# angelvillar96/STLPose

Hardware: AMD Instinct MI355X
Metric: images/sec/GPU HRNet-W32 384x288 train step; PCKh@0.5 parity (higher is better)
Workload: dtype f16/bf16; 1 GPU; HRNet-W32 384x288 bs=32/GPU train step (fwd+MSE+bwd+Adam), random-init weights; global_batch=32, parallelism=dp1

## Files before the change

stlpose_amd/csrc/elementwise.hip:

```cpp
#include "common.cuh"

namespace {

template <typename T>
__device__ __forceinline__ void load8(const void* base, size_t elem, float* f) {
    if constexpr (sizeof(T) == 2) {
        unpack<T>(ldg16((const char*)base + elem * 2), f);
    } else {
        unpack<float>(ldg16((const char*)base + elem * 4), f);
        unpack<float>(ldg16((const char*)base + elem * 4 + 16), f + 4);
    }
}
template <typename T>
__device__ __forceinline__ void store8(void* base, size_t elem, const float* f) {
    if constexpr (sizeof(T) == 2) {
        stg16((char*)base + elem * 2, pack<T>(f));
    } else {
        stg16((char*)base + elem * 4, pack<float>(f));
        stg16((char*)base + elem * 4 + 16, pack<float>(f + 4));
    }
}

template <int NS>
__device__ __forceinline__ void flush_sets(float (*acc)[8], float* red, int C, int VPC, double* const* dst,
// ... 209 lines not shown
                if (t < p.nbn) {
#pragma unroll
                    for (int j = 0; j < 8; ++j)
                        acc[1 + t][j] += d[j] * (y[t][j] - mu[(t * 2) * C + c0 + j]) * mu[(t * 2 + 1) * C + c0 + j];
                }
            }
        }
    }
    if (p.nbn > 0) {
        double* dst[5];
        int which[5];
#pragma unroll
        for (int t = 0; t < 4; ++t) {
            if (t < p.nbn) {
                dst[0] = p.rstats[t], which[0] = 0;
                dst[1] = p.rstats[t], which[1] = 1;
                float two[2][8];
#pragma unroll
                for (int j = 0; j < 8; ++j) two[0][j] = acc[0][j], two[1][j] = acc[1 + t][j];
                flush_sets<2>(two, red, C, VPC, dst, which, 2);
            }
        }
    }
}

template <typename T, typename TY, int SHIFT>
__global__ __launch_bounds__(256) void upsample_bwd_kernel(const stl_upbwd p) {
    extern __shared__ __attribute__((aligned(16))) char smem[];
    const int C = p.C, VPC = C >> 3;
    float* mu = reinterpret_cast<float*>(smem);
    float* red = mu + 2 * C;
    for (int c = threadIdx.x; c < C; c += blockDim.x) {
        float m, r;
        bn_mean_rstd(p.bn, c, C, m, r);
        mu[c] = m, mu[C + c] = r;
    }
    __syncthreads();
    float acc[2][8];
#pragma unroll
    for (int s = 0; s < 2; ++s)
#pragma unroll
        for (int j = 0; j < 8; ++j) acc[s][j] = 0.f;
    constexpr int F = 1 << SHIFT;
    const uint32_t Wh = (uint32_t)p.W << SHIFT, Hh = (uint32_t)p.H << SHIFT;
    const uint32_t total = (uint32_t)p.B * p.H * p.W * VPC;
    const int cg = threadIdx.x % VPC, c0 = cg * 8;
    for (uint32_t v = blockIdx.x * blockDim.x + threadIdx.x; v < total; v += gridDim.x * blockDim.x) {
        const uint32_t pi = v / (uint32_t)VPC;
        const uint32_t by = pi / (uint32_t)p.W, x = pi - by * p.W;
        const uint32_t b = by / (uint32_t)p.H, y = by - b * p.H;
        float yv[8];
        load8<TY>(p.bn.x, (size_t)pi * C + c0, yv);
        float s[8];
#pragma unroll
        for (int j = 0; j < 8; ++j) s[j] = 0.f;
        const size_t row0 = ((size_t)(b * Hh + y * F) * Wh + x * F) * C + c0;
#pragma unroll(SHIFT == 1 ? 2 : 1)
        for (int dy = 0; dy < F; ++dy) {
            float d[F][8];
#pragma unroll
            for (int dx = 0; dx < F; ++dx) load8<T>(p.du, row0 + ((size_t)dy * Wh + dx) * C, d[dx]);
#pragma unroll
            for (int dx = 0; dx < F; ++dx)
#pragma unroll
                for (int j = 0; j < 8; ++j) s[j] += d[dx][j];
        }
#pragma unroll
        for (int j = 0; j < 8; ++j) s[j] = round_to<T>(s[j]);
        store8<T>(p.dt, (size_t)pi * C + c0, s);
#pragma unroll
        for (int j = 0; j < 8; ++j) {
            acc[0][j] += s[j];
            acc[1][j] += s[j] * (yv[j] - mu[c0 + j]) * mu[C + c0 + j];
        }
    }
    double* dst[2] = {p.rstats, p.rstats};
    int which[2] = {0, 1};
    flush_sets<2>(acc, red, C, VPC, dst, which, 2);
}

template <typename T>
__global__ __launch_bounds__(256) void patch_kernel(const float* img, void* out, int B, int H, int W, int Ho, int Wo,
                                                    int stride, const float* mean3, const float* std3) {
    const size_t total = (size_t)B * Ho * Wo * 4;
    float mean[3] = {0.f, 0.f, 0.f}, istd[3] = {1.f, 1.f, 1.f};
    if (mean3) {
#pragma unroll
        for (int c = 0; c < 3; ++c) mean[c] = mean3[c], istd[c] = 1.f / std3[c];
    }
    for (size_t v = (size_t)blockIdx.x * 256 + threadIdx.x; v < total; v += (size_t)gridDim.x * 256) {
        const size_t pi = v >> 2;
        const int part = (int)(v & 3);
        const int ox = (int)(pi % Wo);
        const size_t by = pi / Wo;
        const int oy = (int)(by % Ho), b = (int)(by / Ho);
        float f[8];
#pragma unroll
        for (int j = 0; j < 8; ++j) {
            const int kk = part * 8 + j;
            float val = 0.f;
            if (kk < 27) {
                const int tap = kk / 3, c = kk - tap * 3;
                const int iy = oy * stride + tap / 3 - 1, ix = ox * stride + tap % 3 - 1;
                if (iy >= 0 && iy < H && ix >= 0 && ix < W) {
                    val = img[(((size_t)b * 3 + c) * H + iy) * W + ix];
                    if (mean3) val = (val - mean[c]) / std3[c];
                }
            }
            f[j] = val;
        }
        (void)istd;
        store8<T>(out, pi * 32 + part * 8, f);
    }
}

template <typename T, int S>
__global__ __launch_bounds__(256) void patch_bwd_kernel(const void* dp, float* dimg, int B, int H, int W, int Ho, int Wo,
                                                        const float* std3) {
    constexpr int R0 = S == 1 ? -1 : 0;
    const size_t total = (size_t)B * Ho * Wo;
    for (size_t pi = (size_t)blockIdx.x * 256 + threadIdx.x; pi < total; pi += (size_t)gridDim.x * 256) {
        const int ox = (int)(pi % Wo);
        const size_t by = pi / Wo;
        const int oy = (int)(by % Ho), b = (int)(by / Ho);
        float acc[3][S][S];
#pragma unroll
        for (int c = 0; c < 3; ++c)
#pragma unroll
            for (int u = 0; u < S; ++u)
#pragma unroll
                for (int v = 0; v < S; ++v) acc[c][u][v] = 0.f;
#pragma unroll
        for (int ry = R0; ry <= 1; ++ry) {
#pragma unroll
            for (int rx = R0; rx <= 1; ++rx) {
                const int qy = oy + ry, qx = ox + rx;
                if (qy < 0 || qy >= Ho || qx < 0 || qx >= Wo) continue;
                const size_t row = (((size_t)b * Ho + qy) * Wo + qx) * 32;
                float f[32];
#pragma unroll
                for (int q = 0; q < 4; ++q) load8<T>(dp, row + q * 8, f + q * 8);
#pragma unroll
                for (int ky = 0; ky < 3; ++ky) {
                    const int dy = ry * S + ky - 1;
                    if (dy < 0 || dy >= S) continue;
#pragma unroll
                    for (int kx = 0; kx < 3; ++kx) {
                        const int dx = rx * S + kx - 1;
                        if (dx < 0 || dx >= S) continue;
#pragma unroll
                        for (int c = 0; c < 3; ++c) acc[c][dy][dx] += f[(ky * 3 + kx) * 3 + c];
                    }
                }
            }
        }
#pragma unroll
        for (int c = 0; c < 3; ++c) {
            const float sd = std3 ? std3[c] : 1.f;
#pragma unroll
            for (int u = 0; u < S; ++u) {
                const int iy = oy * S + u;
                if (iy >= H) continue;
                float* dst = dimg + (((size_t)b * 3 + c) * H + iy) * W + (size_t)ox * S;
                if (S == 2 && (W & 1) == 0) {
                    *reinterpret_cast<float2*>(dst) = make_float2(acc[c][u][0] / sd, acc[c][u][S - 1] / sd);
                } else {
#pragma unroll
                    for (int v = 0; v < S; ++v)
                        if (ox * S + v < W) dst[v] = acc[c][u][v] / sd;
                }
            }
        }
    }
}

template <typename T, int J>
__global__ __launch_bounds__(256) void head_fwd_kernel(const void* x, const float* w, const float* bias, float* out,
                                                       int B, int HW, int Ci) {
    extern __shared__ __attribute__((aligned(16))) char smem[];
    float* sw = reinterpret_cast<float*>(smem);
    for (int e = threadIdx.x; e < J * Ci; e += 256) sw[e] = w[e];
    __syncthreads();
    const size_t P = (size_t)B * HW;
    for (size_t pi = (size_t)blockIdx.x * 256 + threadIdx.x; pi < P; pi += (size_t)gridDim.x * 256) {
        float o[J];
#pragma unroll
        for (int j = 0; j < J; ++j) o[j] = bias ? bias[j] : 0.f;
        for (int c0 = 0; c0 < Ci; c0 += 8) {
            float f[8];
            load8<T>(x, pi * Ci + c0, f);
#pragma unroll
            for (int j = 0; j < J; ++j)
#pragma unroll
                for (int q = 0; q < 8; ++q) o[j] = fmaf(f[q], sw[j * Ci + c0 + q], o[j]);
        }
        const size_t b = pi / HW, hw = pi - b * HW;
#pragma unroll
        for (int j = 0; j < J; ++j) out[(b * J + j) * HW + hw] = o[j];
    }
}

template <typename T, int J, typename TY = T>
__global__ __launch_bounds__(256) void head_bwd_kernel(const void* x, const float* w, const float* dout, void* dx,
                                                       float* partial, int B, int HW, int Ci) {
    extern __shared__ __attribute__((aligned(16))) char smem[];
    constexpr int SDP = 260;
    constexpr int NTMAX = 4;
    float* sw = reinterpret_cast<float*>(smem);
    float* sd = sw + ((J * Ci + 3) & ~3);
    float* sx = sd + J * SDP;
    const int tid = threadIdx.x, lane = tid & 63, wave = tid >> 6, r16 = lane & 15, g = lane >> 4;
    const int nt_n = Ci >> 4;
    for (int e = tid; e < J * Ci; e += 256) sw[e] = w[e];
    const int nel = J * Ci + J;
    f32x4 acc[2][NTMAX];
#pragma unroll
    for (int mt = 0; mt < 2; ++mt)
#pragma unroll
        for (int nt = 0; nt < NTMAX; ++nt) acc[mt][nt] = f32x4{0.f, 0.f, 0.f, 0.f};
    float bsum = 0.f;
    const size_t P = (size_t)B * HW;
    const size_t nchunk = (P + 255) / 256;
    for (size_t ch = blockIdx.x; ch < nchunk; ch += gridDim.x) {
        const size_t pi = ch * 256 + tid;
        __syncthreads();
        float d[J];
        if (pi < P) {
            const size_t b = pi / HW, hw = pi - b * HW;
#pragma unroll
            for (int j = 0; j < J; ++j) d[j] = dout[(b * J + j) * HW + hw];
        } else {
#pragma unroll
            for (int j = 0; j < J; ++j) d[j] = 0.f;
        }
#pragma unroll
        for (int j = 0; j < J; ++j) sd[j * SDP + tid] = d[j];
        for (int c0 = 0; c0 < Ci; c0 += 8) {
            float f[8], gx[8];
            if (pi < P) {
                load8<TY>(x, pi * Ci + c0, f);
            } else {
#pragma unroll
                for (int q = 0; q < 8; ++q) f[q] = 0.f;
            }
#pragma unroll
            for (int q = 0; q < 8; ++q) {
                sx[tid * (Ci + 1) + c0 + q] = f[q];
                float s = 0.f;
#pragma unroll
                for (int j = 0; j < J; ++j) s = fmaf(d[j], sw[j * Ci + c0 + q], s);
                gx[q] = s;
            }
            if (pi < P) store8<T>(dx, pi * Ci + c0, gx);
        }
        __syncthreads();
        const int px0 = wave * 64 + g;
        const float* arow0 = sd + r16 * SDP + px0;
        const float* arow1 = sd + (16 + r16 < J ? 16 + r16 : 0) * SDP + px0;
        const bool a1ok = 16 + r16 < J;
        const float* brow = sx + (size_t)px0 * (Ci + 1) + r16;
#pragma unroll 4
        for (int ks = 0; ks < 16; ++ks) {
            const float a0 = arow0[4 * ks];
            const float a1 = a1ok ? arow1[4 * ks] : 0.f;
#pragma unroll
            for (int nt = 0; nt < NTMAX; ++nt) {
                if (nt < nt_n) {
                    const float bv = brow[(size_t)4 * ks * (Ci + 1) + nt * 16];
                    acc[0][nt] = __builtin_amdgcn_mfma_f32_16x16x4f32(a0, bv, acc[0][nt], 0, 0, 0);
                    acc[1][nt] = __builtin_amdgcn_mfma_f32_16x16x4f32(a1, bv, acc[1][nt], 0, 0, 0);
                }
            }
        }
        if (tid < 4 * J) {
            const float* r = sd + (tid >> 2) * SDP + (tid & 3) * 64;
            float s = 0.f;
#pragma unroll
            for (int q = 0; q < 16; ++q) {
                const float4 v = *reinterpret_cast<const float4*>(r + 4 * q);
                s += (v.x + v.y) + (v.z + v.w);
            }
            bsum += s;
        }
    }
    __syncthreads();
    f32x4* red = reinterpret_cast<f32x4*>(sx);
#pragma unroll
    for (int mt = 0; mt < 2; ++mt)
#pragma unroll
        for (int nt = 0; nt < NTMAX; ++nt)
            if (nt < nt_n) red[(wave * 2 * NTMAX + mt * NTMAX + nt) * 64 + lane] = acc[mt][nt];
    float* bred = reinterpret_cast<float*>(red + 4 * 2 * NTMAX * 64);
    if (tid < 4 * J) bred[tid] = bsum;
    __syncthreads();
    for (int e = tid; e < nel; e += 256) {
        float s;
        if (e < J * Ci) {
            const int j = e / Ci, c = e - j * Ci;
            const int tile = (j >> 4) * NTMAX + (c >> 4), ln = 16 * ((j & 15) >> 2) + (c & 15), rr = j & 3;
            s = (red[(0 * 2 * NTMAX + tile) * 64 + ln][rr] + red[(1 * 2 * NTMAX + tile) * 64 + ln][rr]) +
                (red[(2 * 2 * NTMAX + tile) * 64 + ln][rr] + red[(3 * 2 * NTMAX + tile) * 64 + ln][rr]);
        } else {
            const int j = e - J * Ci;
            s = (bred[4 * j] + bred[4 * j + 1]) + (bred[4 * j + 2] + bred[4 * j + 3]);
        }
        partial[(size_t)blockIdx.x * nel + e] = s;
    }
}

__global__ __launch_bounds__(256) void mse_kernel(const float* o, const float* t, const float* tw, float* dout,
                                                  double* partial, size_t n, int HW, float gs) {
    double acc = 0.0;
    for (size_t i = (size_t)blockIdx.x * 256 + threadIdx.x; i < n; i += (size_t)gridDim.x * 256) {
        const float w = tw[i / HW];
        const float d = (o[i] - t[i]) * w;
        acc += (double)d * (double)d;
        if (dout) dout[i] = d * w * gs;
    }
    __shared__ double sred[4];
    acc = wave_sum_d(acc);
    if ((threadIdx.x & 63) == 0) sred[threadIdx.x >> 6] = acc;
    __syncthreads();
    if (threadIdx.x == 0) partial[blockIdx.x] = sred[0] + sred[1] + sred[2] + sred[3];
}

__global__ __launch_bounds__(256) void sum_partials_kernel(const double* partial, int n, double scale, float* out, int accumulate) {
    double acc = 0.0;
    for (int i = threadIdx.x; i < n; i += 256) acc += partial[i];
    __shared__ double sred[4];
    acc = wave_sum_d(acc);
    if ((threadIdx.x & 63) == 0) sred[threadIdx.x >> 6] = acc;
    __syncthreads();
    if (threadIdx.x == 0) {
        const double s = (sred[0] + sred[1] + sred[2] + sred[3]) * scale;
        out[0] = (float)((accumulate ? (double)out[0] : 0.0) + s);
    }
}

__global__ __launch_bounds__(256) void argmax_kernel(const float* hm, int32_t* idx, float* maxval, float* preds, int H, int W) {
    __shared__ float sv[4];
    __shared__ int si[4];
    const float* row = hm + (size_t)blockIdx.x * H * W;
    float bv;
    int bi;
    block_argmax(row, H * W, bv, bi, sv, si);
    if (threadIdx.x == 0) {
        if (idx) idx[blockIdx.x] = bi;
        maxval[blockIdx.x] = bv;
        const float m = bv > 0.f ? 1.f : 0.f;
        preds[2 * blockIdx.x] = (float)(bi % W) * m;
        preds[2 * blockIdx.x + 1] = (float)(bi / W) * m;
    }
}

__global__ __launch_bounds__(256) void final_preds_kernel(const float* hm, const float* center, const float* scale,
                                                          float* preds, float* maxval, int J, int H, int W) {
    __shared__ float sv[4];
    __shared__ int si[4];
    const float* row = hm + (size_t)blockIdx.x * H * W;
    float bv;
    int bi;
    block_argmax(row, H * W, bv, bi, sv, si);
    if (threadIdx.x == 0) {
        const float m = bv > 0.f ? 1.f : 0.f;
        float cx = (float)(bi % W) * m, cy = (float)(bi / W) * m;
        const int px = (int)floorf(cx + 0.5f), py = (int)floorf(cy + 0.5f);
        if (1 < px && px < W - 1 && 1 < py && py < H - 1) {
            const float dx = row[py * W + px + 1] - row[py * W + px - 1];
            const float dy = row[(py + 1) * W + px] - row[(py - 1) * W + px];
            cx += (dx > 0.f) ? 0.25f : (dx < 0.f ? -0.25f : 0.f);
            cy += (dy > 0.f) ? 0.25f : (dy < 0.f ? -0.25f : 0.f);
        }
        const int b = blockIdx.x / J;
        const double s = (double)W / ((double)scale[2 * b] * 200.0);
        preds[2 * blockIdx.x] = (float)(((double)cx - 0.5 * W) / s + (double)center[2 * b]);
        preds[2 * blockIdx.x + 1] = (float)(((double)cy - 0.5 * H) / s + (double)center[2 * b + 1]);
        maxval[blockIdx.x] = bv;
    }
}

__global__ __launch_bounds__(256) void flip_merge_kernel(const float* a, const float* bf, float* out, const int32_t* perm,
                                                         int J, int H, int W, size_t n) {
    for (size_t i = (size_t)blockIdx.x * 256 + threadIdx.x; i < n; i += (size_t)gridDim.x * 256) {
        const int x = (int)(i % W);
        const size_t r = i / W;
        const int y = (int)(r % H);
        const size_t bj = r / H;
        const int j = (int)(bj % J);
        const size_t b = bj / J;
        const int xs = x > 0 ? x - 1 : 0;
        const float f = bf[((b * J + perm[j]) * H + y) * W + (W - 1 - xs)];
        out[i] = 0.5f * (a[i] + f);
    }
}

__global__ __launch_bounds__(256) void flip_merge_bwd_kernel(const float* g, float* da, float* dbf, const int32_t* perm,
                                                             int J, int H, int W, size_t n) {
    for (size_t i = (size_t)blockIdx.x * 256 + threadIdx.x; i < n; i += (size_t)gridDim.x * 256) {
        const int x = (int)(i % W);
        const size_t r = i / W;
// ... 550 lines not shown
    for (int t = 0; t < p.nterms; ++t) flat = flat && p.t[t].shift == 0;
    const bool big = flat && total >= ((size_t)1 << 21) && ((size_t)grid.x * 256) % (size_t)(p.C / 8) == 0;
#define STL_FUSE(TT)                                                                   \
    do {                                                                               \
        if (big) STL_LAUNCH(fuse_flat_big_kernel<TT>, grid, dim3(256), lds, ST, p);    \
        else STL_LAUNCH(fuse_fwd_kernel<TT>, grid, dim3(256), lds, ST, p);             \
    } while (0)
    if (p.dtype == STL_BF16)
        STL_FUSE(__bf16);
    else if (p.dtype == STL_F16)
        STL_FUSE(f16);
    else
        STL_FUSE(float);
#undef STL_FUSE
    STL_LAUNCH_CHECK("fuse_forward");
    return 0;
}

static int stat_block(int C) {
    const int vpc = C / 8;
    return vpc * (256 / vpc);
}

extern "C" int stl_fuse_backward(const stl_fuse_bwd* pp, void* stream) {
    const stl_fuse_bwd& p = *pp;
    STL_CHECK(p.C % 8 == 0 && p.C > 0 && p.C <= 1024, "fuse_bwd: C=%d", p.C);
    STL_CHECK(p.ngrads >= 1 && p.ngrads <= 4 && p.nbn >= 0 && p.nbn <= 4, "fuse_bwd: ngrads/nbn");
    STL_CHECK(!p.relu || p.z, "fuse_bwd: relu needs z");
    for (int t = 0; t < p.nbn; ++t) STL_CHECK(p.bn[t].x && (p.bn[t].stats || (p.bn[t].rmean && p.bn[t].rvar)) && p.rstats[t], "fuse_bwd: bn term %d incomplete", t);
    const int bd = stat_block(p.C);
    const size_t total = (size_t)p.B * p.H * p.W * (p.C / 8);
    int cap = (int)(total / (size_t)(bd * 16));
    cap = cap < 256 ? 256 : (cap > 1024 ? 1024 : cap);
    int nb = nblocks_for(total, bd, cap);
    const size_t lds = (size_t)(p.nbn > 0 ? p.nbn : 1) * 2 * p.C * 4 + (size_t)bd * 2 * 8 * 4;
    STL_CHECK(p.ydtype == 0 || p.ydtype == p.dtype || (p.dtype == STL_BF16 && p.ydtype == STL_F16), "fuse_bwd: ydtype %d does not go with dtype %d", p.ydtype, p.dtype);
    if (p.dtype == STL_BF16 && p.ydtype == STL_F16)
        STL_LAUNCH((fuse_bwd_kernel<__bf16, f16>), dim3(nb), dim3(bd), lds, ST, p);
    else if (p.dtype == STL_BF16)
        STL_LAUNCH(fuse_bwd_kernel<__bf16>, dim3(nb), dim3(bd), lds, ST, p);
    else
        STL_LAUNCH(fuse_bwd_kernel<float>, dim3(nb), dim3(bd), lds, ST, p);
    STL_LAUNCH_CHECK("fuse_backward");
    return 0;
}

extern "C" int stl_upsample_backward(const stl_upbwd* pp, void* stream) {
    const stl_upbwd& p = *pp;
    STL_CHECK(p.C % 8 == 0 && p.C > 0 && p.C <= 1024, "upsample_bwd: C=%d", p.C);
    STL_CHECK(p.shift >= 1 && p.shift <= 3, "upsample_bwd: shift %d (1 .. 3)", p.shift);
    STL_CHECK(p.du && p.dt && p.bn.x && (p.bn.stats || (p.bn.rmean && p.bn.rvar)) && p.rstats, "upsample_bwd: null pointer");
    const int bd = stat_block(p.C);
    const size_t total = (size_t)p.B * p.H * p.W * (p.C / 8);
    int cap = (int)(total / (size_t)(bd * 16));
    cap = cap < 256 ? 256 : (cap > 1024 ? 1024 : cap);
    int nb = nblocks_for(total, bd, cap);
    const size_t lds = (size_t)2 * p.C * 4 + (size_t)bd * 2 * 8 * 4;
    STL_CHECK(p.ydtype == 0 || p.ydtype == p.dtype || (p.dtype == STL_BF16 && p.ydtype == STL_F16), "upsample_bwd: ydtype %d does not go with dtype %d", p.ydtype, p.dtype);
    STL_CHECK(total * 8 < (1ull << 31) && ((size_t)p.B * (p.H << p.shift) * (p.W << p.shift) * p.C) < (1ull << 32),
              "upsample_bwd: tensors of 2^31 or more elements are not supported (32-bit index arithmetic)");
#define STL_UP(TT, TYY)                                                                                         \
    do {                                                                                                        \
        if (p.shift == 1) STL_LAUNCH((upsample_bwd_kernel<TT, TYY, 1>), dim3(nb), dim3(bd), lds, ST, p);        \
        else if (p.shift == 2) STL_LAUNCH((upsample_bwd_kernel<TT, TYY, 2>), dim3(nb), dim3(bd), lds, ST, p);   \
        else if (p.shift == 3) STL_LAUNCH((upsample_bwd_kernel<TT, TYY, 3>), dim3(nb), dim3(bd), lds, ST, p);   \
        else return stl_set_error("upsample_bwd: shift %d has no instantiation (1 .. 3)", p.shift);             \
    } while (0)
    if (p.dtype == STL_BF16 && p.ydtype == STL_F16)
        STL_UP(__bf16, f16);
    else if (p.dtype == STL_BF16)
        STL_UP(__bf16, __bf16);
    else
        STL_UP(float, float);
#undef STL_UP
    STL_LAUNCH_CHECK("upsample_backward");
    return 0;
}

extern "C" int stl_patch3x3(int dtype, const float* img, void* out, int B, int H, int W, int stride, const float* mean3,
                            const float* std3, void* stream) {
    STL_CHECK(stride == 1 || stride == 2, "patch3x3: stride");
    STL_CHECK(img && out && B > 0 && H > 0 && W > 0, "patch3x3: bad args");
    const int Ho = (H + 2 - 3) / stride + 1, Wo = (W + 2 - 3) / stride + 1;
    const size_t total = (size_t)B * Ho * Wo * 4;
    if (dtype == STL_BF16)
        STL_LAUNCH(patch_kernel<__bf16>, dim3(nblocks_for(total, 256, 4096)), dim3(256), 0, ST, img, out, B, H, W, Ho, Wo, stride, mean3, std3);
    else if (dtype == STL_F16)
        STL_LAUNCH(patch_kernel<f16>, dim3(nblocks_for(total, 256, 4096)), dim3(256), 0, ST, img, out, B, H, W, Ho, Wo, stride, mean3, std3);
    else
        STL_LAUNCH(patch_kernel<float>, dim3(nblocks_for(total, 256, 4096)), dim3(256), 0, ST, img, out, B, H, W, Ho, Wo, stride, mean3, std3);
    STL_LAUNCH_CHECK("patch3x3");
    return 0;
}

extern "C" int stl_patch3x3_backward(int dtype, const void* dpatch, float* dimg, int B, int H, int W, int stride, const float* std3,
                                     void* stream) {
    STL_CHECK(stride == 1 || stride == 2, "patch3x3_backward: stride");
    STL_CHECK(dpatch && dimg && B > 0 && H > 0 && W > 0, "patch3x3_backward: bad args");
    const int Ho = (H + 2 - 3) / stride + 1, Wo = (W + 2 - 3) / stride + 1;
    const size_t total = (size_t)B * Ho * Wo;
    const dim3 grid(nblocks_for(total, 256, 4096));
#define PB(TT)                                                                                                              \
    do {                                                                                                                    \
        if (stride == 2) STL_LAUNCH((patch_bwd_kernel<TT, 2>), grid, dim3(256), 0, ST, dpatch, dimg, B, H, W, Ho, Wo, std3); \
        else STL_LAUNCH((patch_bwd_kernel<TT, 1>), grid, dim3(256), 0, ST, dpatch, dimg, B, H, W, Ho, Wo, std3);            \
    } while (0)
    if (dtype == STL_BF16) PB(__bf16);
    else if (dtype == STL_F16) PB(f16);
    else PB(float);
#undef PB
    STL_LAUNCH_CHECK("patch3x3_backward");
    return 0;
}

extern "C" int stl_head_forward(int dtype, const void* x, const float* w, const float* bias, float* out, int B, int H, int W,
                                int Ci, int J, void* stream) {
    STL_CHECK(J == 17 || J == 16, "head: J=%d unsupported (16 or 17)", J);
    STL_CHECK(Ci % 8 == 0 && Ci <= 512, "head: Ci=%d", Ci);
    const size_t P = (size_t)B * H * W;
    const size_t lds = (size_t)J * Ci * 4;
    const dim3 grid(nblocks_for(P));
#define HF(T, JJ) STL_LAUNCH((head_fwd_kernel<T, JJ>), grid, dim3(256), lds, ST, x, w, bias, out, B, H * W, Ci)
    if (dtype == STL_BF16) { if (J == 17) HF(__bf16, 17); else HF(__bf16, 16); }
    else if (dtype == STL_F16) { if (J == 17) HF(f16, 17); else HF(f16, 16); }
    else { if (J == 17) HF(float, 17); else HF(float, 16); }
#undef HF
    STL_LAUNCH_CHECK("head_forward");
    return 0;
}

extern "C" int stl_head_backward(int dtype2, const void* x, const float* w, const float* dout, void* dx, float* partial,
                                 int nblk, int B, int H, int W, int Ci, int J, void* stream) {
    const int dtype = dtype2 & 0xff, ydtype = (dtype2 >> 8) & 0xff;
    STL_CHECK(ydtype == 0 || ydtype == dtype || (dtype == STL_BF16 && ydtype == STL_F16), "head_bwd: x type %d does not go with dx type %d", ydtype, dtype);
    STL_CHECK(J == 17 || J == 16, "head_bwd: J=%d unsupported", J);
    STL_CHECK(nblk >= 1, "head_bwd: nblk");
    STL_CHECK(Ci % 16 == 0 && Ci <= 64, "head_bwd: Ci=%d must be a multiple of 16, at most 64", Ci);
    size_t lds = (size_t)(((J * Ci + 3) & ~3) + J * 260 + 256 * (Ci + 1)) * 4;
    const size_t lds_red = (size_t)(((J * Ci + 3) & ~3) + J * 260) * 4 + (size_t)4 * 2 * 4 * 64 * 16 + 4 * J * 4;
    if (lds_red > lds) lds = lds_red;
    static bool attr = false;
    if (!attr) {
        hipFuncSetAttribute(reinterpret_cast<const void*>(&head_bwd_kernel<__bf16, 17>), hipFuncAttributeMaxDynamicSharedMemorySize, 160 * 1024);
        hipFuncSetAttribute(reinterpret_cast<const void*>(&head_bwd_kernel<__bf16, 16>), hipFuncAttributeMaxDynamicSharedMemorySize, 160 * 1024);
        hipFuncSetAttribute(reinterpret_cast<const void*>(&head_bwd_kernel<float, 17>), hipFuncAttributeMaxDynamicSharedMemorySize, 160 * 1024);
        hipFuncSetAttribute(reinterpret_cast<const void*>(&head_bwd_kernel<float, 16>), hipFuncAttributeMaxDynamicSharedMemorySize, 160 * 1024);
        hipFuncSetAttribute(reinterpret_cast<const void*>(&head_bwd_kernel<__bf16, 17, f16>), hipFuncAttributeMaxDynamicSharedMemorySize, 160 * 1024);
        hipFuncSetAttribute(reinterpret_cast<const void*>(&head_bwd_kernel<__bf16, 16, f16>), hipFuncAttributeMaxDynamicSharedMemorySize, 160 * 1024);
        attr = true;
    }
#define HB(T, JJ, TY) STL_LAUNCH((head_bwd_kernel<T, JJ, TY>), dim3(nblk), dim3(256), lds, ST, x, w, dout, dx, partial, B, H * W, Ci)
    if (dtype == STL_BF16 && ydtype == STL_F16) { if (J == 17) HB(__bf16, 17, f16); else HB(__bf16, 16, f16); }
    else if (dtype == STL_BF16) { if (J == 17) HB(__bf16, 17, __bf16); else HB(__bf16, 16, __bf16); }
    else { if (J == 17) HB(float, 17, float); else HB(float, 16, float); }
#undef HB
    STL_LAUNCH_CHECK("head_backward");
    return 0;
}

extern "C" int stl_sum_partials(const double* partial, int n, double scale, float* out, int accumulate, void* stream) {
    STL_LAUNCH(sum_partials_kernel, dim3(1), dim3(256), 0, ST, partial, n, scale, out, accumulate);
    STL_LAUNCH_CHECK("sum_partials");
    return 0;
}

extern "C" int stl_mse_loss(const float* out, const float* target, const float* tweight, float* dout, double* partial,
                            int nblk, float* loss, int B, int J, int HW, float gscale, void* stream) {
    STL_CHECK(out && target && tweight && partial && nblk >= 1, "mse: null pointer");
    const size_t n = (size_t)B * J * HW;
    STL_LAUNCH(mse_kernel, dim3(nblk), dim3(256), 0, ST, out, target, tweight, dout, partial, n, HW, gscale / (float)n);
    STL_LAUNCH_CHECK("mse_loss");
    if (!loss) return 0;
    return stl_sum_partials(partial, nblk, 0.5 / (double)n, loss, 0, stream);
}

extern "C" int stl_heatmap_argmax(const float* hm, int32_t* idx, float* maxval, float* preds, int BJ, int H, int W, void* stream) {
    if (BJ == 0) return 0;
    STL_CHECK(hm && maxval && preds && H > 0 && W > 0, "argmax: bad args");
    STL_LAUNCH(argmax_kernel, dim3(BJ), dim3(256), 0, ST, hm, idx, maxval, preds, H, W);
    STL_LAUNCH_CHECK("heatmap_argmax");
    return 0;
}

extern "C" int stl_final_preds(const float* hm, const float* center, const float* scale, float* preds, float* maxval, int B,
                               int J, int H, int W, void* stream) {
    if (B * J == 0) return 0;
    STL_LAUNCH(final_preds_kernel, dim3(B * J), dim3(256), 0, ST, hm, center, scale, preds, maxval, J, H, W);
    STL_LAUNCH_CHECK("final_preds");
    return 0;
}

extern "C" int stl_flip_merge(const float* a, const float* bflip, float* out, const int32_t* perm, int B, int J, int H, int W,
                              void* stream) {
    const size_t n = (size_t)B * J * H * W;
    if (n == 0) return 0;
    STL_LAUNCH(flip_merge_kernel, dim3(nblocks_for(n)), dim3(256), 0, ST, a, bflip, out, perm, J, H, W, n);
    STL_LAUNCH_CHECK("flip_merge");
    return 0;
}

extern "C" int stl_flip_merge_backward(const float* g, float* da, float* dbf, const int32_t* perm, int B, int J, int H, int W,
                                       void* stream) {
    const size_t n = (size_t)B * J * H * W;
    if (n == 0) return 0;
    STL_CHECK(g && da && dbf && perm, "flip_merge_backward: null pointer");
    STL_LAUNCH(flip_merge_bwd_kernel, dim3(nblocks_for(n)), dim3(256), 0, ST, g, da, dbf, perm, J, H, W, n);
    STL_LAUNCH_CHECK("flip_merge_backward");
    return 0;
}

extern "C" int stl_weight_prep(int dtype2, const float* master, void* wk, const stl_wprep* tab, int n, int nblocks, void* stream) {
    if (n == 0 || nblocks == 0) return 0;
    STL_CHECK(master && wk && tab && n > 0 && nblocks > 0, "weight_prep: bad arguments");
    const int dtype = dtype2 & 0xff, fdtype = (dtype2 >> 8) & 0xff;
    STL_CHECK(fdtype == 0 || fdtype == dtype || (dtype == STL_BF16 && fdtype == STL_F16), "weight_prep: forward type %d does not go with %d", fdtype, dtype);
    if (dtype == STL_BF16 && fdtype == STL_F16)
        STL_LAUNCH((weight_prep_kernel<__bf16, f16>), dim3(nblocks), dim3(256), 0, ST, master, (__bf16*)wk, tab, n, 0);
    else if (dtype == STL_F16)
        STL_LAUNCH((weight_prep_kernel<f16, f16>), dim3(nblocks), dim3(256), 0, ST, master, (f16*)wk, tab, n, 0);
    else if (dtype == STL_BF16)
        STL_LAUNCH(weight_prep_kernel<__bf16>, dim3(nblocks), dim3(256), 0, ST, master, (__bf16*)wk, tab, n, 0);
    else
        STL_LAUNCH(weight_prep_kernel<float>, dim3(nblocks), dim3(256), 0, ST, master, (float*)wk, tab, n, 0);
    STL_LAUNCH_CHECK("weight_prep");
    return 0;
}

extern "C" int stl_reduce_slabs(const float* partials, float* grads, const stl_slab* tab, int n, int nblocks, void* stream) {
    if (n == 0) return 0;
    STL_LAUNCH(reduce_slabs_kernel, dim3(nblocks), dim3(256), 0, ST, partials, grads, tab, n, 0);
    STL_LAUNCH_CHECK("reduce_slabs");
    return 0;
}

extern "C" int stl_reduce_slabs_range(const stl_reduce_range* r, void* stream) {
    STL_CHECK(r && r->partials && r->grads && r->tab && r->n >= 0 && r->nblocks >= 0, "reduce_slabs_range: bad arguments");
    if (r->n == 0 || r->nblocks == 0) return 0;
    STL_LAUNCH(reduce_slabs_kernel, dim3(r->nblocks), dim3(256), 0, ST, r->partials, r->grads, r->tab, r->n, r->blk_base);
    STL_LAUNCH_CHECK("reduce_slabs_range");
    return 0;
}

extern "C" int stl_bn_running_update(const double* stats, float* buffers, int64_t* nbt, const stl_bnrec* tab, int n,
                                     float momentum, int32_t* overflow, void* stream) {
    if (n == 0) return 0;
    STL_LAUNCH(bn_running_kernel, dim3(n), dim3(256), 0, ST, stats, buffers, nbt, tab, momentum, overflow);
    STL_LAUNCH_CHECK("bn_running_update");
    return 0;
}

extern "C" int stl_bn_param_grads(const double* rstats, float* grads, const stl_bnrec* tab, int n, void* stream) {
    if (n == 0) return 0;
    STL_LAUNCH(bn_param_grads_kernel, dim3(n), dim3(256), 0, ST, rstats, grads, tab);
// ... 164 lines not shown
```

Measured before the change: 2499 images/sec.

## Vectorize patch, head fwd/bwd and MSE kernels with prefetch and coalesced stores

```diff
diff --git a/stlpose_amd/csrc/elementwise.hip b/stlpose_amd/csrc/elementwise.hip
--- a/stlpose_amd/csrc/elementwise.hip
+++ b/stlpose_amd/csrc/elementwise.hip
@@ -315,35 +315,56 @@
 template <typename T>
 __global__ __launch_bounds__(256) void patch_kernel(const float* img, void* out, int B, int H, int W, int Ho, int Wo,
                                                     int stride, const float* mean3, const float* std3) {
-    const size_t total = (size_t)B * Ho * Wo * 4;
-    float mean[3] = {0.f, 0.f, 0.f}, istd[3] = {1.f, 1.f, 1.f};
+    constexpr int NVP = sizeof(T) == 2 ? 4 : 8;
+    constexpr int EPV = 32 / NVP;
+    constexpr int PITCH = NVP + 1;
+    __shared__ V16 st[256 * PITCH];
+    const uint32_t P = (uint32_t)B * Ho * Wo;
+    float mean[3] = {0.f, 0.f, 0.f}, sd[3] = {1.f, 1.f, 1.f};
     if (mean3) {
 #pragma unroll
-        for (int c = 0; c < 3; ++c) mean[c] = mean3[c], istd[c] = 1.f / std3[c];
-    }
-    for (size_t v = (size_t)blockIdx.x * 256 + threadIdx.x; v < total; v += (size_t)gridDim.x * 256) {
-        const size_t pi = v >> 2;
-        const int part = (int)(v & 3);
-        const int ox = (int)(pi % Wo);
-        const size_t by = pi / Wo;
-        const int oy = (int)(by % Ho), b = (int)(by / Ho);
-        float f[8];
-#pragma unroll
-        for (int j = 0; j < 8; ++j) {
-            const int kk = part * 8 + j;
-            float val = 0.f;
-            if (kk < 27) {
-                const int tap = kk / 3, c = kk - tap * 3;
-                const int iy = oy * stride + tap / 3 - 1, ix = ox * stride + tap % 3 - 1;
-                if (iy >= 0 && iy < H && ix >= 0 && ix < W) {
-                    val = img[(((size_t)b * 3 + c) * H + iy) * W + ix];
-                    if (mean3) val = (val - mean[c]) / std3[c];
+        for (int c = 0; c < 3; ++c) mean[c] = mean3[c], sd[c] = std3[c];
+    }
+    const int plane = H * W;
+    const int tid = threadIdx.x;
+    for (uint32_t p0 = blockIdx.x * 256u; p0 < P; p0 += gridDim.x * 256u) {
+        const uint32_t pi = p0 + tid;
+        if (pi < P) {
+            const uint32_t ox = pi % (uint32_t)Wo, by = pi / (uint32_t)Wo, oy = by % (uint32_t)Ho, b = by / (uint32_t)Ho;
+            const float* ib = img + (size_t)b * 3 * plane;
+            const int iy0 = (int)oy * stride - 1, ix0 = (int)ox * stride - 1;
+            float f[32];
+            bool ok[9];
+#pragma unroll
+            for (int tap = 0; tap < 9; ++tap) {
+                const int iy = iy0 + tap / 3, ix = ix0 + tap % 3;
+                ok[tap] = iy >= 0 && iy < H && ix >= 0 && ix < W;
+                const int off = ok[tap] ? iy * W + ix : 0;
+#pragma unroll
+                for (int c = 0; c < 3; ++c) f[tap * 3 + c] = ib[c * plane + off];
+            }
+#pragma unroll
+            for (int tap = 0; tap < 9; ++tap)
+#pragma unroll
+                for (int c = 0; c < 3; ++c) {
+                    float val = f[tap * 3 + c];
+                    if (mean3) val = (val - mean[c]) / sd[c];
+                    f[tap * 3 + c] = ok[tap] ? val : 0.f;
                 }
-            }
-            f[j] = val;
-        }
-        (void)istd;
-        store8<T>(out, pi * 32 + part * 8, f);
+#pragma unroll
+            for (int kk = 27; kk < 32; ++kk) f[kk] = 0.f;
+#pragma unroll
+            for (int v = 0; v < NVP; ++v) st[tid * PITCH + v] = pack<T>(f + v * EPV);
+        }
+        __syncthreads();
+        const uint32_t nvec = (P - p0 < 256u ? P - p0 : 256u) * NVP;
+        char* dst = (char*)out + (size_t)p0 * NVP * 16;
+#pragma unroll
+        for (int k = 0; k < NVP; ++k) {
+            const uint32_t idx = k * 256 + tid;
+            if (idx < nvec) stg16(dst + (size_t)idx * 16, st[(idx / NVP) * PITCH + idx % NVP]);
+        }
+        __syncthreads();
     }
 }
 
@@ -407,14 +428,75 @@
     }
 }
 
+template <typename T, int NV>
+struct HeadPixel {
+    static constexpr int NR = NV * (sizeof(T) == 4 ? 2 : 1);
+    V16 raw[NR];
+    __device__ __forceinline__ void load(const void* x, size_t pi) {
+        const char* p = (const char*)x + pi * (size_t)(NR * 16);
+#pragma unroll
+        for (int v = 0; v < NR; ++v) raw[v] = ldg16(p + v * 16);
+    }
+    __device__ __forceinline__ void vec8(int v, float* f) const {
+        if constexpr (sizeof(T) == 2) {
+            unpack<T>(raw[v], f);
+        } else {
+            unpack<float>(raw[2 * v], f);
+            unpack<float>(raw[2 * v + 1], f + 4);
+        }
+    }
+};
+
+template <typename T, int J, int NV>
+__device__ __forceinline__ void head_fwd_pixels(const void* x, const float* w, const float* bias, float* out, size_t P, int HW, float* sw0) {
+    constexpr int Ci = NV * 8;
+    HeadPixel<T, NV> px;
+    size_t pi = (size_t)blockIdx.x * 256 + threadIdx.x;
+    bool have = pi < P;
+    if (have) px.load(x, pi);
+    for (int e = threadIdx.x; e < J * Ci; e += 256) sw0[e] = w[e];
+    float bj[J];
+#pragma unroll
+    for (int j = 0; j < J; ++j) bj[j] = bias ? bias[j] : 0.f;
+    __syncthreads();
+    while (have) {
+        int off = 0;
+        asm volatile("" : "+v"(off));
+        const float* sw = sw0 + off;
+        const size_t b = pi / HW, hw = pi - b * HW;
+        float* dst = out + b * J * HW + hw;
+        float o[J];
+#pragma unroll
+        for (int j = 0; j < J; ++j) o[j] = bj[j];
+#pragma unroll
+        for (int v = 0; v < NV; ++v) {
+            __builtin_amdgcn_sched_barrier(0);
+            float f[8];
+            px.vec8(v, f);
+#pragma unroll
+            for (int j = 0; j < J; ++j)
+#pragma unroll
+                for (int q = 0; q < 8; ++q) o[j] = fmaf(f[q], sw[j * Ci + v * 8 + q], o[j]);
+        }
+#pragma unroll
+        for (int j = 0; j < J; ++j) dst[(size_t)j * HW] = o[j];
+        pi += (size_t)gridDim.x * 256;
+        have = pi < P;
+        if (have) px.load(x, pi);
+    }
+}
+
 template <typename T, int J>
 __global__ __launch_bounds__(256) void head_fwd_kernel(const void* x, const float* w, const float* bias, float* out,
                                                        int B, int HW, int Ci) {
     extern __shared__ __attribute__((aligned(16))) char smem[];
     float* sw = reinterpret_cast<float*>(smem);
+    const size_t P = (size_t)B * HW;
+    if (Ci == 32) return head_fwd_pixels<T, J, 4>(x, w, bias, out, P, HW, sw);
+    if (Ci == 48) return head_fwd_pixels<T, J, 6>(x, w, bias, out, P, HW, sw);
+    if (Ci == 64) return head_fwd_pixels<T, J, 8>(x, w, bias, out, P, HW, sw);
     for (int e = threadIdx.x; e < J * Ci; e += 256) sw[e] = w[e];
     __syncthreads();
-    const size_t P = (size_t)B * HW;
     for (size_t pi = (size_t)blockIdx.x * 256 + threadIdx.x; pi < P; pi += (size_t)gridDim.x * 256) {
         float o[J];
 #pragma unroll
@@ -433,18 +515,18 @@
     }
 }
 
-template <typename T, int J, typename TY = T>
-__global__ __launch_bounds__(256) void head_bwd_kernel(const void* x, const float* w, const float* dout, void* dx,
-                                                       float* partial, int B, int HW, int Ci) {
-    extern __shared__ __attribute__((aligned(16))) char smem[];
+template <typename T, int J, typename TY, int NV>
+__device__ __forceinline__ void head_bwd_body(const void* x, const float* w, const float* dout, void* dx, float* partial, size_t P,
+                                              int HW, char* smem) {
+    constexpr int Ci = NV * 8;
     constexpr int SDP = 260;
     constexpr int NTMAX = 4;
+    constexpr int nt_n = Ci >> 4;
+    constexpr int PX = Ci + 4;
     float* sw = reinterpret_cast<float*>(smem);
     float* sd = sw + ((J * Ci + 3) & ~3);
     float* sx = sd + J * SDP;
     const int tid = threadIdx.x, lane = tid & 63, wave = tid >> 6, r16 = lane & 15, g = lane >> 4;
-    const int nt_n = Ci >> 4;
-    for (int e = tid; e < J * Ci; e += 256) sw[e] = w[e];
     const int nel = J * Ci + J;
     f32x4 acc[2][NTMAX];
 #pragma unroll
@@ -452,57 +534,78 @@
 #pragma unroll
         for (int nt = 0; nt < NTMAX; ++nt) acc[mt][nt] = f32x4{0.f, 0.f, 0.f, 0.f};
     float bsum = 0.f;
-    const size_t P = (size_t)B * HW;
     const size_t nchunk = (P + 255) / 256;
+    const bool small = P <= 0xFFFFFFFFull;
+    HeadPixel<TY, NV> nx;
+    float dn[J];
+    auto request = [&](size_t ch) {
+        const size_t pi = ch * 256 + tid;
+        if (pi < P) {
+            size_t b, hw;
+            if (small) {
+                const uint32_t b32 = (uint32_t)pi / (uint32_t)HW;
+                b = b32, hw = (uint32_t)pi - b32 * (uint32_t)HW;
+            } else {
+                b = pi / HW, hw = pi - b * HW;
+            }
+            const float* dp = dout + b * J * HW + hw;
+#pragma unroll
+            for (int j = 0; j < J; ++j) dn[j] = dp[(size_t)j * HW];
+            nx.load(x, pi);
+        } else {
+#pragma unroll
+            for (int j = 0; j < J; ++j) dn[j] = 0.f;
+#pragma unroll
+            for (int v = 0; v < HeadPixel<TY, NV>::NR; ++v) nx.raw[v] = zero16();
+        }
+    };
+    if (blockIdx.x < nchunk) request(blockIdx.x);
+    for (int e = tid; e < J * Ci; e += 256) sw[e] = w[e];
+    float* const sxrow = sx + ((tid & ~7) | ((tid & 1) << 2) | ((tid & 7) >> 1)) * PX;
     for (size_t ch = blockIdx.x; ch < nchunk; ch += gridDim.x) {
         const size_t pi = ch * 256 + tid;
         __syncthreads();
         float d[J];
+#pragma unroll
+        for (int j = 0; j < J; ++j) d[j] = dn[j], sd[j * SDP + tid] = d[j];
+#pragma unroll
+        for (int v = 0; v < NV; ++v) {
+            float f[8];
+            nx.vec8(v, f);
+            *reinterpret_cast<float4*>(sxrow + v * 8) = make_float4(f[0], f[1], f[2], f[3]);
+            *reinterpret_cast<float4*>(sxrow + v * 8 + 4) = make_float4(f[4], f[5], f[6], f[7]);
+        }
         if (pi < P) {
-            const size_t b = pi / HW, hw = pi - b * HW;
-#pragma unroll
-            for (int j = 0; j < J; ++j) d[j] = dout[(b * J + j) * HW + hw];
-        } else {
-#pragma unroll
-            for (int j = 0; j < J; ++j) d[j] = 0.f;
-        }
-#pragma unroll
-        for (int j = 0; j < J; ++j) sd[j * SDP + tid] = d[j];
-        for (int c0 = 0; c0 < Ci; c0 += 8) {
-            float f[8], gx[8];
-            if (pi < P) {
-                load8<TY>(x, pi * Ci + c0, f);
-            } else {
-#pragma unroll
-                for (int q = 0; q < 8; ++q) f[q] = 0.f;
-            }
-#pragma unroll
-            for (int q = 0; q < 8; ++q) {
-                sx[tid * (Ci + 1) + c0 + q] = f[q];
-                float s = 0.f;
-#pragma unroll
-                for (int j = 0; j < J; ++j) s = fmaf(d[j], sw[j * Ci + c0 + q], s);
-                gx[q] = s;
-            }
-            if (pi < P) store8<T>(dx, pi * Ci + c0, gx);
-        }
+#pragma unroll
+            for (int v = 0; v < NV; ++v) {
+                __builtin_amdgcn_sched_barrier(0);
+                float gx[8];
+#pragma unroll
+                for (int q = 0; q < 8; ++q) {
+                    float s = 0.f;
+#pragma unroll
+                    for (int j = 0; j < J; ++j) s = fmaf(d[j], sw[j * Ci + v * 8 + q], s);
+                    gx[q] = s;
+                }
+                store8<T>(dx, pi * Ci + v * 8, gx);
+            }
+        }
+        if (ch + gridDim.x < nchunk) request(ch + gridDim.x);
         __syncthreads();
         const int px0 = wave * 64 + g;
         const float* arow0 = sd + r16 * SDP + px0;
         const float* arow1 = sd + (16 + r16 < J ? 16 + r16 : 0) * SDP + px0;
         const bool a1ok = 16 + r16 < J;
-        const float* brow = sx + (size_t)px0 * (Ci + 1) + r16;
+        const float* brow = sx + (wave * 64 + ((g & 1) << 2) + (g >> 1)) * PX + r16;
 #pragma unroll 4
         for (int ks = 0; ks < 16; ++ks) {
             const float a0 = arow0[4 * ks];
             const float a1 = a1ok ? arow1[4 * ks] : 0.f;
 #pragma unroll
-            for (int nt = 0; nt < NTMAX; ++nt) {
-                if (nt < nt_n) {
-                    const float bv = brow[(size_t)4 * ks * (Ci + 1) + nt * 16];
-                    acc[0][nt] = __builtin_amdgcn_mfma_f32_16x16x4f32(a0, bv, acc[0][nt], 0, 0, 0);
-                    acc[1][nt] = __builtin_amdgcn_mfma_f32_16x16x4f32(a1, bv, acc[1][nt], 0, 0, 0);
-                }
+            for (int nt = 0; nt < nt_n; ++nt) {
+                const float bv = brow[(8 * (ks >> 1) + 2 * (ks & 1)) * PX + nt * 16];
+                acc[0][nt] = __builtin_amdgcn_mfma_f32_16x16x4f32(a0, bv, acc[0][nt], 0, 0, 0);
+                acc[1][nt] = __builtin_amdgcn_mfma_f32_16x16x4f32(a1, bv, acc[1][nt], 0, 0, 0);
             }
         }
         if (tid < 4 * J) {
@@ -541,14 +644,65 @@
     }
 }
 
+template <typename T, int J, typename TY = T>
+__global__ __launch_bounds__(256) void head_bwd_kernel(const void* x, const float* w, const float* dout, void* dx,
+                                                       float* partial, int B, int HW, int Ci) {
+    extern __shared__ __attribute__((aligned(16))) char smem[];
+    const size_t P = (size_t)B * HW;
+    switch (Ci) {
+        case 16: return head_bwd_body<T, J, TY, 2>(x, w, dout, dx, partial, P, HW, smem);
+        case 32: return head_bwd_body<T, J, TY, 4>(x, w, dout, dx, partial, P, HW, smem);
+        case 48: return head_bwd_body<T, J, TY, 6>(x, w, dout, dx, partial, P, HW, smem);
+        default: return head_bwd_body<T, J, TY, 8>(x, w, dout, dx, partial, P, HW, smem);
+    }
+}
+
+__device__ __forceinline__ float mse_elem(float o, float t, float w, float gs, double& acc) {
+    const float d = (o - t) * w;
+    acc += (double)d * (double)d;
+    return d * w * gs;
+}
+
+constexpr int MSE_U = 4;
 __global__ __launch_bounds__(256) void mse_kernel(const float* o, const float* t, const float* tw, float* dout,
-                                                  double* partial, size_t n, int HW, float gs) {
+                                                  double* partial, size_t n, int HW, float gs, uint32_t rcp) {
     double acc = 0.0;
-    for (size_t i = (size_t)blockIdx.x * 256 + threadIdx.x; i < n; i += (size_t)gridDim.x * 256) {
-        const float w = tw[i / HW];
-        const float d = (o[i] - t[i]) * w;
-        acc += (double)d * (double)d;
-        if (dout) dout[i] = d * w * gs;
+    const bool vec = n < ((size_t)1 << 31) && HW >= 4 && (((uintptr_t)o | (uintptr_t)t | (uintptr_t)dout) & 15) == 0;
+    if (vec) {
+        const uint32_t nv = (uint32_t)(n >> 2), hw = (uint32_t)HW;
+        for (size_t v0 = (size_t)blockIdx.x * (256 * MSE_U) + threadIdx.x; v0 < nv; v0 += (size_t)gridDim.x * (256 * MSE_U)) {
+            float4 a[MSE_U], b[MSE_U];
+            float w0[MSE_U], w1[MSE_U];
+            uint32_t left[MSE_U];
+#pragma unroll
+            for (int u = 0; u < MSE_U; ++u) {
+                const uint32_t v = (uint32_t)v0 + u * 256, vv = v < nv ? v : (uint32_t)v0;
+                a[u] = *reinterpret_cast<const float4*>(o + (size_t)vv * 4);
+                b[u] = *reinterpret_cast<const float4*>(t + (size_t)vv * 4);
+                const uint32_t i = vv * 4;
+                uint32_t q = __umulhi(i, rcp), r = i - q * hw;
+                if (r >= hw) ++q, r -= hw;
+                left[u] = hw - r;
+                w0[u] = tw[q];
+                w1[u] = tw[q + (left[u] < 4 ? 1u : 0u)];
+            }
+#pragma unroll
+            for (int u = 0; u < MSE_U; ++u) {
+                const uint32_t v = (uint32_t)v0 + u * 256;
+                if (v < nv) {
+                    float4 g;
+                    g.x = mse_elem(a[u].x, b[u].x, w0[u], gs, acc);
+                    g.y = mse_elem(a[u].y, b[u].y, left[u] > 1 ? w0[u] : w1[u], gs, acc);
+                    g.z = mse_elem(a[u].z, b[u].z, left[u] > 2 ? w0[u] : w1[u], gs, acc);
+                    g.w = mse_elem(a[u].w, b[u].w, left[u] > 3 ? w0[u] : w1[u], gs, acc);
+                    if (dout) *reinterpret_cast<float4*>(dout + (size_t)v * 4) = g;
+                }
+            }
+        }
+    }
+    for (size_t i = (vec ? (n & ~(size_t)3) : 0) + (size_t)blockIdx.x * 256 + threadIdx.x; i < n; i += (size_t)gridDim.x * 256) {
+        const float g = mse_elem(o[i], t[i], tw[i / HW], gs, acc);
+        if (dout) dout[i] = g;
     }
     __shared__ double sred[4];
     acc = wave_sum_d(acc);
@@ -1265,13 +1419,15 @@
     STL_CHECK(stride == 1 || stride == 2, "patch3x3: stride");
     STL_CHECK(img && out && B > 0 && H > 0 && W > 0, "patch3x3: bad args");
     const int Ho = (H + 2 - 3) / stride + 1, Wo = (W + 2 - 3) / stride + 1;
-    const size_t total = (size_t)B * Ho * Wo * 4;
+    const size_t total = (size_t)B * Ho * Wo;
+    STL_CHECK(total < ((size_t)1 << 31) && (size_t)3 * H * W < ((size_t)1 << 31), "patch3x3: 2^31 or more pixels are not supported (32-bit index arithmetic)");
+    const dim3 grid(nblocks_for(total, 256, 4096));
     if (dtype == STL_BF16)
-        STL_LAUNCH(patch_kernel<__bf16>, dim3(nblocks_for(total, 256, 4096)), dim3(256), 0, ST, img, out, B, H, W, Ho, Wo, stride, mean3, std3);
+        STL_LAUNCH(patch_kernel<__bf16>, grid, dim3(256), 0, ST, img, out, B, H, W, Ho, Wo, stride, mean3, std3);
     else if (dtype == STL_F16)
-        STL_LAUNCH(patch_kernel<f16>, dim3(nblocks_for(total, 256, 4096)), dim3(256), 0, ST, img, out, B, H, W, Ho, Wo, stride, mean3, std3);
+        STL_LAUNCH(patch_kernel<f16>, grid, dim3(256), 0, ST, img, out, B, H, W, Ho, Wo, stride, mean3, std3);
     else
-        STL_LAUNCH(patch_kernel<float>, dim3(nblocks_for(total, 256, 4096)), dim3(256), 0, ST, img, out, B, H, W, Ho, Wo, stride, mean3, std3);
+        STL_LAUNCH(patch_kernel<float>, grid, dim3(256), 0, ST, img, out, B, H, W, Ho, Wo, stride, mean3, std3);
     STL_LAUNCH_CHECK("patch3x3");
     return 0;
 }
@@ -1319,7 +1475,7 @@
     STL_CHECK(J == 17 || J == 16, "head_bwd: J=%d unsupported", J);
     STL_CHECK(nblk >= 1, "head_bwd: nblk");
     STL_CHECK(Ci % 16 == 0 && Ci <= 64, "head_bwd: Ci=%d must be a multiple of 16, at most 64", Ci);
-    size_t lds = (size_t)(((J * Ci + 3) & ~3) + J * 260 + 256 * (Ci + 1)) * 4;
+    size_t lds = (size_t)(((J * Ci + 3) & ~3) + J * 260 + 256 * (Ci + 4)) * 4;
     const size_t lds_red = (size_t)(((J * Ci + 3) & ~3) + J * 260) * 4 + (size_t)4 * 2 * 4 * 64 * 16 + 4 * J * 4;
     if (lds_red > lds) lds = lds_red;
     static bool attr = false;
@@ -1351,7 +1507,8 @@
                             int nblk, float* loss, int B, int J, int HW, float gscale, void* stream) {
     STL_CHECK(out && target && tweight && partial && nblk >= 1, "mse: null pointer");
     const size_t n = (size_t)B * J * HW;
-    STL_LAUNCH(mse_kernel, dim3(nblk), dim3(256), 0, ST, out, target, tweight, dout, partial, n, HW, gscale / (float)n);
+    const uint32_t rcp = HW > 1 ? (uint32_t)(((uint64_t)1 << 32) / (uint32_t)HW) : 0xFFFFFFFFu;
+    STL_LAUNCH(mse_kernel, dim3(nblk), dim3(256), 0, ST, out, target, tweight, dout, partial, n, HW, gscale / (float)n, rcp);
     STL_LAUNCH_CHECK("mse_loss");
     if (!loss) return 0;
     return stl_sum_partials(partial, nblk, 0.5 / (double)n, loss, 0, stream);
```

Result: no change. 2499 images/sec (+0.0%).
